# TheEconomist/us-potus-model

Hardware: AMD Instinct MI355X
Metric: leapfrog_steps_per_sec (higher is better)
Workload: dtype f64

## Files before the change

### us_potus_model_amd/csrc/potus_cluster.hpp

```cpp
#pragma once
#include "potus_nuts.hpp"
#include "potus_dpp.hpp"

#define CL_MAXDAYS 64
#define CL_MAXK 32
#define CL_DW4_MAXAVG 26
#define CL_AUX_SC1 16
#define CL_NCHUNK PT_NW
#define CL_SEG_SHIFT 64
#define CL_SPIN_LIMIT 8000000u
#ifndef CL_SPIN_SLEEP
#define CL_SPIN_SLEEP 1
#endif

enum { CP_D0 = 0, CP_ND, CP_P0, CP_NP, CP_E0, CP_NE, CP_R0, CP_NR, CP_NSUB, CP_NSEG, CP_WB,
       CP_O_WD, CP_O_MASK, CP_O_SUB, CP_O_SEGPTR, CP_O_SEGKIND, CP_O_SEGIDX, CP_O_WT, CP_E_SH, CP_NCELL, CP_O_CELL, CP_N = 24 };
#define CL_CELLS_PER_THREAD 2
#define CL_G_PAD 16
enum { XP_PRE = 0, XP_AR = 64, XP_S = 66, XP_P = 72 };
enum { XQ0 = 64 };

struct ClModel {
  int K, XW, NR, NREP, NDP, npmax, nsubmax, Dint;
  const int *part;
  const int *sched;
  const double *wt;
  const int *rep_pos;
  const int *rep_owner;
  const double *rep_scale;
  const int *perm;
  int GS, GROWS;
  int l_C, l_G, l_Lw, l_prior, l_pm, l_py, l_pun, l_sub, l_tab, l_ru, l_wide, l_wout, l_X, l_Y, l_r, l_rep, l_bT, l_e, l_c1, l_c2, l_c3, l_ge, l_P, l_scal, l_red, l_st, l_prof;
  int lds_doubles;
};
typedef const ClModel AS_C *CCp;

#define CL_WIDE 96
struct ClLay {
  int l_C, l_G, l_Lw, l_prior, l_pm, l_py, l_pun, l_sub, l_tab, l_ru, l_wide, l_wout, l_X, l_Y, l_r, l_rep, l_bT, l_e, l_c1, l_c2, l_c3, l_ge, l_P, l_scal, l_red, l_st, l_prof;
  int l_rm, l_rpf, l_rrs;
  int total;
};
constexpr int cl_ev(int n) { return (n + 1) & ~1; }
constexpr ClLay cl_layout(int S, int SE, int SP, int NDP, int npcap, int nsubcap, int nrepcap, int nrcap, int tcap, int g_doubles, int necap = 0) {
  ClLay L{};
  int o = 0;
  L.l_C = o; o += cl_ev(S * NDP);
  L.l_G = g_doubles ? o : 0; o += cl_ev(g_doubles);
  L.l_Lw = o; o += cl_ev((SE + 1) * SP);
  L.l_prior = o; o += cl_ev(SE);
  L.l_pm = o; o += cl_ev(npcap + 8);
  L.l_py = o; o += cl_ev(npcap + 8);
  L.l_pun = o; o += cl_ev(npcap + 8);
  L.l_sub = o; o += cl_ev(nsubcap * 4 + 4);
  L.l_tab = o; o += cl_ev((npcap + 64) / 2 + 2);
  L.l_ru = o; o += cl_ev(npcap + 2);
  L.l_wide = o; o += cl_ev(CL_WIDE * PT_NW);
  L.l_wout = o; o += cl_ev(CL_WIDE);
  L.l_X = o; o += cl_ev((PT_NW + 1) * SE);
  L.l_Y = o; o += cl_ev((PT_NW + 1) * SE > nsubcap ? (PT_NW + 1) * SE : nsubcap);
  L.l_r = o; o += cl_ev(npcap + 2);
  L.l_rep = o; o += cl_ev(nrepcap + 2);
  L.l_bT = o; o += cl_ev(SE);
  L.l_e = o; o += cl_ev(tcap);
  L.l_c1 = o; o += cl_ev(CL_MAXDAYS);
  L.l_c2 = o; o += cl_ev(CL_MAXDAYS);
  L.l_c3 = o; o += cl_ev(CL_MAXDAYS);
  L.l_ge = o; o += cl_ev(CL_MAXDAYS);
  L.l_P = o; o += cl_ev(nrcap + 8);
  L.l_scal = o; o += cl_ev(SC_N);
  L.l_red = o; o += cl_ev((PT_NW + 1) * PT_NRED);
  L.l_st = o; o += cl_ev((npcap + 8 + 7) / 8);
  L.l_prof = o; o += cl_ev(PT_NPROF);
  L.l_rm = necap ? o : 0; o += necap ? cl_ev(necap + 8) : 0;
  L.l_rpf = necap ? o : 0; o += necap ? cl_ev(necap + 8) : 0;
  L.l_rrs = necap ? o : 0; o += necap ? cl_ev(necap + 8) : 0;
  L.total = o;
  return L;
}

struct ClFixed {
  static constexpr int S = 51, SE = 52, SP = 51, NDP = 33;
  static constexpr int NPCAP = 256, NSUBCAP = 384, NREPCAP = 768, NRCAP = 512, TCAP = 320;
  static constexpr int KMAX = 16;
  static constexpr int NECAP = 1920;
  static constexpr int XW = 832;
  static constexpr int GS = 48, GROWS = 52;
  static constexpr ClLay L = cl_layout(S, SE, SP, NDP, NPCAP, NSUBCAP, NREPCAP, NRCAP, TCAP, 0, NECAP);
#define CLF(f) static constexpr int f = L.f
  CLF(l_C); CLF(l_G); CLF(l_Lw); CLF(l_prior); CLF(l_pm); CLF(l_py); CLF(l_pun); CLF(l_sub); CLF(l_tab); CLF(l_ru); CLF(l_wide); CLF(l_wout); CLF(l_X); CLF(l_Y);
  CLF(l_r); CLF(l_rep); CLF(l_bT); CLF(l_e); CLF(l_c1); CLF(l_c2); CLF(l_c3); CLF(l_ge); CLF(l_P); CLF(l_scal); CLF(l_red); CLF(l_st); CLF(l_prof); CLF(l_rm); CLF(l_rpf); CLF(l_rrs);
#undef CLF
  static constexpr int lds_doubles = L.total;
};
template <int TAG> struct ClTag {
  static constexpr int DW = (TAG == 12 || TAG == 16 || TAG == 17) ? 4 : TAG;
  static constexpr bool MF = TAG == 12;
  static constexpr bool FX = TAG == 16 || TAG == 17;
  static constexpr int FULL = TAG == 16 ? 1 : 0;
};
typedef const int AS_C *cip;

__device__ __forceinline__ double bld_s(rsrc_t r, unsigned voff, unsigned soff) {
  return __builtin_bit_cast(double, __builtin_amdgcn_raw_buffer_load_b64(r, voff, soff, CL_AUX_SC1));
}
__device__ __forceinline__ void bst_s(rsrc_t r, unsigned voff, unsigned soff, double v) {
  __builtin_amdgcn_raw_buffer_store_b64(__builtin_bit_cast(u32x2, v), r, voff, soff, CL_AUX_SC1);
}
__device__ __forceinline__ double readlane_d(double v, int l) {
  const unsigned long long u = __builtin_bit_cast(unsigned long long, v);
  const unsigned lo = __builtin_amdgcn_readlane((unsigned)u, l), hi = __builtin_amdgcn_readlane((unsigned)(u >> 32), l);
  return __builtin_bit_cast(double, ((unsigned long long)hi << 32) | lo);
}
template <class P> __device__ __forceinline__ P launder_s(P p) {
  unsigned lo = __builtin_amdgcn_readfirstlane((unsigned)(unsigned long long)p);
  unsigned hi = __builtin_amdgcn_readfirstlane((unsigned)((unsigned long long)p >> 32));
  asm volatile("" : "+s"(lo), "+s"(hi));
  return (P)(((unsigned long long)hi << 32) | lo);
}

#ifdef POTUS_PROF
#define PROFPTR prof
#define CPROFPTR(c) (c).prof
#else
#define PROFPTR nullptr
#define CPROFPTR(c) nullptr
#endif
#if defined(POTUS_PROF_FETCH) && (POTUS_PROF_FETCH + 0) == 2
#define XPROF_A(p) nullptr
#define XPROF_B(p) (p)
#elif defined(POTUS_PROF_FETCH)
#define XPROF_A(p) (p)
#define XPROF_B(p) nullptr
#else
#define XPROF_A(p) nullptr
#define XPROF_B(p) nullptr
#endif
__shared__ int cl_dead;
__shared__ int cl_local;
#define STORE128_PAD(w) asm volatile("s_nop 1" :: "v"(w) : "memory")
struct Xch {
  rsrc_t xb;
  unsigned epoch;
  unsigned launch;
  unsigned x1e;
  int K, m, XW;
  int local;
};
__device__ __forceinline__ unsigned xch_wslot(const Xch &x, int mm) { return ((((x.epoch + 1u) & 3u) * (unsigned)x.K + (unsigned)mm) * (unsigned)x.XW) * 16u; }
__device__ __forceinline__ unsigned xch_rslot(const Xch &x, int mm) { return (((x.epoch & 3u) * (unsigned)x.K + (unsigned)mm) * (unsigned)x.XW) * 16u; }
__device__ __forceinline__ unsigned xch_eslot(const Xch &x, unsigned e, int mm) { return (((e & 3u) * (unsigned)x.K + (unsigned)mm) * (unsigned)x.XW) * 16u; }
__device__ __forceinline__ unsigned xch_wdoff(const Xch &x) { return 4u * (unsigned)x.K * (unsigned)x.XW * 16u; }
__device__ __forceinline__ bool xch_watchdog_raised(const Xch &x) {
  return __builtin_amdgcn_readfirstlane(__builtin_amdgcn_raw_buffer_load_b32(x.xb, 0u, __builtin_amdgcn_readfirstlane(xch_wdoff(x)), CL_AUX_SC1)) != 0u;
}
__device__ __forceinline__ void xch_give_up(const Xch &x) {
  __builtin_amdgcn_raw_buffer_store_b32(1u, x.xb, 0u, __builtin_amdgcn_readfirstlane(xch_wdoff(x)), CL_AUX_SC1);
  cl_dead = 1;
  asm volatile("s_waitcnt vmcnt(0) lgkmcnt(0)" ::: "memory");
  __builtin_amdgcn_endpgm();
}
__device__ __forceinline__ void xst(const Xch &x, unsigned voff, double v) {
  const unsigned long long u = __builtin_bit_cast(unsigned long long, v);
  const u32x4 w = {(unsigned)u, (unsigned)(u >> 32), x.epoch + 1u, x.launch};
  const unsigned so = __builtin_amdgcn_readfirstlane(xch_wslot(x, x.m));
  __builtin_amdgcn_raw_buffer_store_b128(w, x.xb, x.local ? voff : PT_OOB, so, 0);
  __builtin_amdgcn_raw_buffer_store_b128(w, x.xb, x.local ? PT_OOB : voff, so, CL_AUX_SC1);
  STORE128_PAD(w);
}
template <int NB>
__device__ __forceinline__ bool xld(const Xch &x_in, const unsigned (&vo)[NB], const unsigned (&so)[NB], double (&out)[NB], unsigned tag = 0, ldp xprof = nullptr) {
  Xch x = x_in;
  if (tag) x.epoch = tag;
  x.epoch = __builtin_amdgcn_readfirstlane(x.epoch); x.launch = __builtin_amdgcn_readfirstlane(x.launch);
#ifdef POTUS_PROF_FETCH
  const long long xt0_ = clock64();
#else
  (void)xprof;
#endif
  u32x4 w[NB];
  bool done[NB];
  unsigned ss[NB];
#pragma unroll
  for (int u = 0; u < NB; u++) ss[u] = __builtin_amdgcn_readfirstlane(so[u]);
// ... 242 lines not shown
  static constexpr int NEXTRA = 3;
  double extra[3];
  struct QT { double q; };
  struct GT { double p, m, pp; };
  __device__ __forceinline__ void q_load(unsigned vo, QT &t) { t.q = bld(r, vo, sQc); }
  __device__ __forceinline__ void qs_load(unsigned vo, QT &t) { t.q = bld_s(r, vo, sQc); }
  __device__ __forceinline__ double q_fin(QT &t) { return t.q; }
  __device__ __forceinline__ void g_load(unsigned vo, GT &t) {
    t.p = bld(r, vo, sPH); t.m = bld(r, vo, sM);
    t.pp = bld(r, fuse1 ? vo : PT_OOB, sPrev);
  }
  template <bool SHARED>
  __device__ __forceinline__ double fin(unsigned vo, double v, double q, const GT &t) {
    const double pf = t.p + he * v;
    bst(r, vo, sL, pf);
    const double ph = pf + he * v;
    bst(r, vo, sPH, ph);
    const double qn = q + e * t.m * ph;
    if (SHARED) bst_s(r, vo, sQn, qn);
    else bst(r, vo, sQn, qn);
    const double rs = t.pp + pf;
    bst(r, fuse1 ? vo : PT_OOB, sOut1, rs);
    extra[0] += t.m * pf * pf;
    extra[1] += t.m * t.pp * rs;
    extra[2] += t.m * pf * rs;
    return qn;
  }
  __device__ __forceinline__ double g_fin(unsigned vo, double v, double q, const GT &t) { return fin<false>(vo, v, q, t); }
  __device__ __forceinline__ double gs_fin(unsigned vo, double v, double q, const GT &t) { return fin<true>(vo, v, q, t); }
};

struct ClLeapPolicyRes {
  rsrc_t r;
  unsigned sQc, sQn, sPH, sL;
  double he, e;
  unsigned sOut1;
  bool fuse1, out1_global;
  unsigned e0b;
  static constexpr int NEXTRA = 3;
  double extra[3];
  struct QT { double q; };
  struct GT { double p, m, pp; };
  __device__ __forceinline__ int slot(unsigned vo) const { return vo == PT_OOB ? (int)ClFixed::NECAP : (int)((vo - e0b) >> 3); }
  static __device__ __forceinline__ ldp RM() { return (ldp)lds_dyn + ClFixed::l_rm; }
  static __device__ __forceinline__ ldp RPF() { return (ldp)lds_dyn + ClFixed::l_rpf; }
  static __device__ __forceinline__ ldp RRS() { return (ldp)lds_dyn + ClFixed::l_rrs; }
  __device__ __forceinline__ void q_load(unsigned vo, QT &t) { t.q = bld(r, vo, sQc); }
  __device__ __forceinline__ void qs_load(unsigned vo, QT &t) { t.q = bld_s(r, vo, sQc); }
  __device__ __forceinline__ double q_fin(QT &t) { return t.q; }
  __device__ __forceinline__ void g_load(unsigned vo, GT &t) {
    t.p = bld(r, vo, sPH);
    const int idx = slot(vo);
    t.m = RM()[idx];
    const double ppv = RPF()[idx];
    t.pp = fuse1 ? ppv : 0.0;
  }
  template <bool SHARED>
  __device__ __forceinline__ double fin(unsigned vo, double v, double q, const GT &t) {
    const int idx = slot(vo);
    const bool ok = vo != PT_OOB;
    const double pf = t.p + he * v;
    bst(r, vo, sL, pf);
    RPF()[idx] = ok ? pf : 0.0;
    const double ph = pf + he * v;
    bst(r, vo, sPH, ph);
    const double qn = q + e * t.m * ph;
    if (SHARED) bst_s(r, vo, sQn, qn);
    else bst(r, vo, sQn, qn);
    const double rs = t.pp + pf;
    RRS()[idx] = ok ? rs : 0.0;
    bst(r, (fuse1 && out1_global) ? vo : PT_OOB, sOut1, rs);
    extra[0] += t.m * pf * pf;
    extra[1] += t.m * t.pp * rs;
    extra[2] += t.m * pf * rs;
    return qn;
  }
  __device__ __forceinline__ double g_fin(unsigned vo, double v, double q, const GT &t) { return fin<false>(vo, v, q, t); }
  __device__ __forceinline__ double gs_fin(unsigned vo, double v, double q, const GT &t) { return fin<true>(vo, v, q, t); }
};

struct ClStatic {
  int s2info;
  int wd0, wnd;
  int ca, cb;
  unsigned rep_vo[2];
  unsigned rep_xo[2];
  int sg_a, sg_b, sg_kind, sg_index;
  double scale_r;
  int cellw[CL_CELLS_PER_THREAD];
};

__device__ __forceinline__ ClStatic cl_load_static(CCp CL, cip part) {
  ClStatic c;
  gcip sc = as_g(CL->sched) + part[CP_O_WD];
  const int tid = threadIdx.x;
  c.s2info = sc[tid];
  c.wd0 = sc[PT_THREADS + (tid >> 6)]; c.wnd = sc[PT_THREADS + PT_NW + (tid >> 6)];
  c.ca = sc[PT_THREADS + 2 * PT_NW + (tid >> 6)]; c.cb = sc[PT_THREADS + 3 * PT_NW + (tid >> 6)];
  gcip rp = as_g(CL->rep_pos);
  const int NREP = CL->NREP;
  gcip ro = as_g(CL->rep_owner);
#pragma unroll
  for (int u = 0; u < 2; u++) {
    const int j = tid + u * PT_THREADS;
    c.rep_vo[u] = j < NREP ? 8u * (unsigned)rp[j] : PT_OOB;
    c.rep_xo[u] = j < NREP ? ((unsigned)ro[j] * (unsigned)CL->XW + (unsigned)(XQ0 + j)) * 16u : PT_OOB;
  }
  {
    gcip sch = as_g(CL->sched);
    const int nseg = part[CP_NSEG];
    const int sg = CL->l_G ? ((tid + PT_THREADS / 2) & (PT_THREADS - 1)) : ((tid + PT_THREADS - CL_SEG_SHIFT) & (PT_THREADS - 1));
    const bool ok = sg < nseg;
    c.sg_a = ok ? sch[part[CP_O_SEGPTR] + sg] : 0;
    c.sg_b = ok ? sch[part[CP_O_SEGPTR] + sg + 1] : 0;
    c.sg_kind = ok ? sch[part[CP_O_SEGKIND] + sg] : 3;
    c.sg_index = ok ? sch[part[CP_O_SEGIDX] + sg] : 0;
#pragma unroll
    for (int h = 0; h < CL_CELLS_PER_THREAD; h++) c.cellw[h] = CL->l_G ? sch[part[CP_O_CELL] + h * PT_THREADS + tid] : 0;
    const int jr = tid - 128;
    c.scale_r = (jr >= 0 && jr < part[CP_NR]) ? as_g(CL->rep_scale)[part[CP_R0] + jr] : 0.0;
  }
  return c;
}
__device__ __forceinline__ ClStatic cl_setup_lds(CMp M, CCp CL, cip part, ldp lds) {
  if (threadIdx.x == 0) { cl_dead = 0; cl_local = 0; }
#ifdef CL_POISON_LDS
  for (int i = threadIdx.x; i < CL->lds_doubles; i += PT_THREADS) lds[i] = __builtin_nan("");
  __syncthreads();
#endif
  ldp Lw = lds + CL->l_Lw;
  gcdp src = as_g(M->mat);
  for (int i = threadIdx.x; i < (M->SE + 1) * M->SP; i += PT_THREADS) Lw[i] = i < M->SE * M->SP ? src[i] : 0.0;
  for (int i = threadIdx.x; i < M->SE; i += PT_THREADS) (lds + CL->l_prior)[i] = src[M->m_priorx + i];
  unsigned char AS_L *st = (unsigned char AS_L *)(lds + CL->l_st);
  gcip ps = as_g(M->pi) + part[CP_P0];
  const int np = part[CP_NP];
  for (int i = threadIdx.x; i < np + 8; i += PT_THREADS) st[i] = i < np ? (unsigned char)ps[i] : (unsigned char)0;
  {
    unsigned long long AS_L *pm = (unsigned long long AS_L *)(lds + CL->l_pm);
    unsigned long long AS_L *pyn = (unsigned long long AS_L *)(lds + CL->l_py);
    ldp pun = lds + CL->l_pun;
    const int Npad = M->Npad, p0 = part[CP_P0], d0 = part[CP_D0], full = M->full;
    gcip pi = as_g(M->pi);
    gcdp pd = as_g(M->pd);
    for (int i = threadIdx.x; i < np + 8; i += PT_THREADS) {
      unsigned long long v = 0;
      double y = 0.0, N = 0.0, un = 0.0;
      if (i < np) {
        const int g = p0 + i;
        v = (unsigned long long)(unsigned)pi[g] | ((unsigned long long)(unsigned)(pi[Npad + g] - d0) << 8) |
            ((unsigned long long)(unsigned)pi[2 * Npad + g] << 16);
        if (full) v |= ((unsigned long long)(unsigned)pi[3 * Npad + g] << 32) | ((unsigned long long)(unsigned)pi[4 * Npad + g] << 40);
        {
          gcip scw = as_g(CL->sched) + part[CP_O_WD];
          const int tl_ = pi[Npad + g] - d0;
          int wt = 0;
          for (int w_ = 0; w_ < PT_NW; w_++) { const int a_ = scw[PT_THREADS + w_], n_ = scw[PT_THREADS + PT_NW + w_]; if (tl_ >= a_ && tl_ < a_ + n_) wt = w_; }
          v |= (unsigned long long)(unsigned)wt << 48;
        }
        y = pd[g]; N = pd[Npad + g]; un = full ? pd[2 * Npad + g] : 0.0;
      }
      pm[i] = v; pyn[i] = (unsigned long long)(unsigned)(int)y | ((unsigned long long)(unsigned)(int)N << 32); pun[i] = un;
    }
    unsigned AS_L *tab = (unsigned AS_L *)(lds + CL->l_tab);
    gcip src_tab = as_g(CL->sched) + part[CP_O_MASK];
    for (int i = threadIdx.x; i < np + 64; i += PT_THREADS) tab[i] = i < np ? (unsigned)src_tab[i] : 0u;
    unsigned short AS_L *sb = (unsigned short AS_L *)(lds + CL->l_sub);
    gcip src_sub = as_g(CL->sched) + part[CP_O_SUB];
    const int n16 = part[CP_NSUB] * PT_SUBLEN;
    for (int i = threadIdx.x; i < n16; i += PT_THREADS) sb[i] = (unsigned short)src_sub[i];
  }
  if (CL->l_G) for (int i = threadIdx.x; i < CL->GROWS * CL->GS + CL_G_PAD; i += PT_THREADS) (lds + CL->l_G)[i] = 0.0;
  const ClStatic c = cl_load_static(CL, part);
#ifdef POTUS_PROF
  for (int i = threadIdx.x; i < PT_NPROF; i += PT_THREADS) (lds + CL->l_prof)[i] = 0.0;
#endif
  __syncthreads();
  return c;
}

__device__ __forceinline__ int uni_i(int v) { return __builtin_amdgcn_readfirstlane(v); }

template <int CL_TAG, class Pol>
__device__ __forceinline__ double cl_pass_partial(CMp M_in, CCp CL_in, cip part_in, ldp lds, const ClStatic &cst, Xch &x, Pol &pol_io,
                                                  bool pubnext, const LeafCtx &pend, ltp ts, ldp wout, bool &aborted) {
  constexpr int CL_DW = ClTag<CL_TAG>::DW;
  constexpr bool MF = ClTag<CL_TAG>::MF, FX = ClTag<CL_TAG>::FX;
#define LAY(f) (FX ? (int)ClFixed::f : CL->f)
  Pol pol = pol_io;
  int tid = threadIdx.x;
  asm volatile("" : "+v"(tid));
  CMp M = launder_s(M_in);
  CCp CL = launder_s(CL_in);
  cip part = launder_s(part_in);
  const int lane = tid & 63;
  const int w = __builtin_amdgcn_readfirstlane(tid >> 6);
  if constexpr (FX) lds = (ldp)lds_dyn;
  const int S = FX ? (int)ClFixed::S : M->S, T = M->T, SE = FX ? (int)ClFixed::SE : M->SE, SP = FX ? (int)ClFixed::SP : M->SP, full = FX ? ClTag<CL_TAG>::FULL : M->full, o_c = M->o_c;
  const int NDP = FX ? (int)ClFixed::NDP : CL->NDP, NR = CL->NR, NREP = CL->NREP;
  const int d0 = part[CP_D0], nd = part[CP_ND], np = part[CP_NP], e0 = part[CP_E0], r0 = part[CP_R0], nr = part[CP_NR];
  const int K = x.K, m = x.m;
  const int wd0 = __builtin_amdgcn_readfirstlane(cst.wd0), wnd = __builtin_amdgcn_readfirstlane(cst.wnd);
  ldp C = lds + LAY(l_C), Lw = lds + LAY(l_Lw), X = lds + LAY(l_X), Y = lds + LAY(l_Y), r_lds = lds + LAY(l_r), ru_lds = lds + LAY(l_ru);
  ldp s_rep = lds + LAY(l_rep);
  ldp s_zT = s_rep, s_zb = s_rep + S, s_mid = s_rep + 2 * S;
  ldp s_bT = lds + LAY(l_bT), s_e = lds + LAY(l_e), s_c1 = lds + LAY(l_c1), s_c2 = lds + LAY(l_c2), s_c3 = lds + LAY(l_c3);
  ldp s_ge = lds + LAY(l_ge), s_P = lds + LAY(l_P), s_scal = lds + LAY(l_scal), red = lds + LAY(l_red);
  const int e_noise = e0 + S * nd, e_ze = part[CP_E_SH], e_rep = e_ze + (full ? nd : 0);
  double lp = 0.0;
#ifdef POTUS_PROF
  ldp prof = lds + LAY(l_prof);
#endif
  PROF_START();
  TSTAMP(0);

  double cs[CL_DW], zq[CL_DW];
  {
    typename Pol::QT qr[2], qt[CL_DW];
    const bool ahead = x.x1e != 0;
    pol.qs_load(ahead ? PT_OOB : cst.rep_vo[0], qr[0]);
    pol.qs_load(ahead ? PT_OOB : cst.rep_vo[1], qr[1]);
    double qx[2];
    {
      const unsigned vo[2] = {ahead ? cst.rep_xo[0] : PT_OOB, ahead ? cst.rep_xo[1] : PT_OOB};
      const unsigned so[2] = {xch_eslot(x, x.x1e, 0), xch_eslot(x, x.x1e, 0)};
      xld(x, vo, so, qx, ahead ? x.x1e : 1u);
    }
#pragma unroll
    for (int j = 0; j < CL_DW; j++) {
      const int tl = wd0 + j;
      pol.q_load((lane < S && j < wnd) ? 8u * (unsigned)(e0 + lane + S * tl) : PT_OOB, qt[j]);
    }
    for (int i = tid; i < NR + 8; i += PT_THREADS) s_P[i] = 0.0;
    if (tid >= 64 && tid < 64 + CL_MAXDAYS) s_ge[tid - 64] = 0.0;
#pragma unroll
    for (int u = 0; u < 2; u++) { const int j = tid + u * PT_THREADS; s_rep[j < NREP ? j : NREP] = ahead ? qx[u] : pol.q_fin(qr[u]); }
    double run = 0.0;
#pragma unroll
    for (int j = CL_DW - 1; j >= 0; j--) {
      const int t = d0 + wd0 + j;
      const double z = pol.q_fin(qt[j]);
      zq[j] = z;
      lp -= 0.5 * z * z;
      run += (t < T - 1) ? z : 0.0;
      cs[j] = run;
    }
    if (lane < S) {
      Y[w * SE + lane] = run;
#pragma unroll
      for (int j = 0; j < CL_DW; j++) { if (j < wnd) C[lane * NDP + wd0 + j] = cs[j]; }
    }
  }
  __syncthreads();
// ... 144 lines not shown
      s_scal[SC_DSRHO] = M->sigma_e * (-rho / sqrt(1.0 - rho * rho));
    }
    if (w == PT_NW - 2 && pend.n >= 0) {
      WPROF_T0B();
      WPROF_PTB(29);
      cl_leaf_logic(ts, pend, wout);
      WPROF_PTB(30);
    }
    const bool no_polls_here = w == PT_NW - 2 && pend.n >= 0 && np <= 64 * w;
    for (int i0 = 0; i0 < (no_polls_here ? 0 : np); i0 += PT_THREADS) {
      const int il = i0 + tid;
      const bool ok = il < np, lead = ok;
      const int ic = ok ? il : np;
      const unsigned vq = lead ? 8u * (unsigned)(e_noise + il) : PT_OOB;
      typename Pol::QT qt;
      typename Pol::GT gt;
      pol.q_load(vq, qt);
      pol.g_load(vq, gt);
      double gval = 0.0, zn = 0.0;
      if (i0 + 64 * w < np) {
        const unsigned long long meta = pm[ic];
        const int s = (int)(meta & 0xffu), tl = (int)((meta >> 8) & 0xffu), ip = (int)((meta >> 16) & 0xffffu);
        const int im = (int)((meta >> 32) & 0xffu), ipop = (int)((meta >> 40) & 0xffu);
        const unsigned long long yn = pyn[ic];
        const double y = (double)(int)(unsigned)yn, N = (double)(int)(unsigned)(yn >> 32), un = pun[ic];
        const int t = d0 + tl;
        ldp L0 = Lw + s * SP, C0 = C + tl, CW = X + (int)((meta >> 48) & 0xffu) * SE;
        double a0 = 0.0, a1 = 0.0;
          int k0 = 0;
          constexpr int DW_ = 10;
          for (; k0 + DW_ <= S; k0 += DW_) {
            double l[DW_], c[DW_], cw[DW_];
#pragma unroll
            for (int j = 0; j < DW_; j++) { l[j] = L0[k0 + j]; c[j] = C0[(k0 + j) * NDP]; cw[j] = CW[k0 + j]; }
            ISSUE_FENCE();
#pragma unroll
            for (int j = 0; j < DW_; j++) c[j] = c[j] + cw[j];
#pragma unroll
            for (int j = 0; j < DW_; j += 2) { a0 += l[j] * c[j]; a1 += l[j + 1] * c[j + 1]; }
          }
          for (; k0 < S; k0 += 4) {
            double l[4], c[4];
#pragma unroll
            for (int j = 0; j < 4; j++) { const int kk = min(k0 + j, S - 1); l[j] = L0[kk]; c[j] = C0[kk * NDP] + CW[kk]; }
            ISSUE_FENCE();
#pragma unroll
            for (int j = 0; j < 4; j += 2) {
              a0 += (k0 + j < S ? l[j] : 0.0) * c[j];
              a1 += (k0 + j + 1 < S ? l[j + 1] : 0.0) * c[j + 1];
            }
          }
        const double dot = a0 + a1;
        const double sg = s == S ? sigma_nn : sigma_ns;
        WPROF_CSTAMP(0);
        zn = pol.q_fin(qt);
#if (POTUS_PROF_CMASK & 2)
        __builtin_amdgcn_s_waitcnt(0x0F70);
#endif
        WPROF_CSTAMP(1);
        double eta = s_bT[s] + sg * zn + sigma_c * s_mid[ip] + dot;
        if (full) eta += sigma_m * s_mid[om + im] + sigma_pop * s_mid[opop + ipop] + un * s_e[t];
        const double ex = exp(-fabs(eta)), l1 = log1p(ex), pr = (eta >= 0.0 ? 1.0 : ex) / (1.0 + ex);
        const double r = y - N * pr;
        WPROF_CSTAMP(2);
        const double term = y * (fmin(eta, 0.0) - l1) + (N - y) * (fmin(-eta, 0.0) - l1) - 0.5 * zn * zn;
        lp += term;
        r_lds[lead ? il : np + 1] = r;
        ru_lds[lead ? il : np + 1] = r * un;
        gval = sg * r - zn;
      }
      pol.g_fin(vq, gval, zn, gt);
      WPROF_CSTAMP(3);
    }
    WPROF_CFLUSH();
  }
  WAVE_ARRIVE(3);
  __syncthreads();
  PROF_MARK(3);
  TSTAMP(4);
  if (pend.n >= 0 && uni_i(ts->abort)) { aborted = true; return 0.0; }

  if constexpr (!MF) {
    const unsigned AS_L *tab = (const unsigned AS_L *)(lds + LAY(l_tab));
    const int lk = lane < S ? lane : 0;
    const int ca = __builtin_amdgcn_readfirstlane(cst.ca), cb = __builtin_amdgcn_readfirstlane(cst.cb);
    double acc = 0.0;
    for (int base = ca; base < cb; base += 64) {
      const int mine = base + lane < cb ? base + lane : np;
      const unsigned ev = tab[mine];
      const double rv = r_lds[mine];
      const int cnt = min(64, cb - base);
      for (int p0 = 0; p0 < cnt; p0 += 8) {
        unsigned e8[8];
        double r8[8], l8[8];
#pragma unroll
        for (int u = 0; u < 8; u++) {
          const int pu = p0 + u;
          e8[u] = (unsigned)__builtin_amdgcn_readlane((int)ev, pu);
          r8[u] = readlane_d(rv, pu);
          l8[u] = Lw[(int)(e8[u] & 0xffu) * SP + lk];
        }
        ISSUE_FENCE();
#pragma unroll
        for (int u = 0; u < 8; u++) {
          acc += r8[u] * l8[u];
          if (e8[u] & 0x10000u) {
            if (lane < S) C[lane * NDP + (int)((e8[u] >> 8) & 0xffu)] = acc;
          }
        }
      }
    }
    if (lane < S) X[w * SE + lane] = acc;
  }
  if constexpr (MF) {
    ldp G = lds + LAY(l_G);
#pragma unroll
    for (int h = 0; h < CL_CELLS_PER_THREAD; h++) {
      if (h == 0 || part[CP_NCELL] > h * PT_THREADS) {
        const int cw = cst.cellw[h], a = cw & 1023, cnt = (cw >> 10) & 63, off = (int)((unsigned)cw >> 16);
        double sum = r_lds[a];
        for (int i = 1; i < cnt; i++) sum += r_lds[a + i];
        G[off] = sum;
      }
    }
  }
  {
    const int nsub = part[CP_NSUB], wb = part[CP_WB];
    const u32x4 AS_L *sb = (const u32x4 AS_L *)(lds + LAY(l_sub));
    for (int sub0 = 0; sub0 < nsub; sub0 += PT_THREADS) {
      const int sub = sub0 + tid;
      const bool ok = sub < nsub;
      const u32x4 ia = sb[ok ? 2 * sub : 0], ib = sb[ok ? 2 * sub + 1 : 0];
      double rr[PT_SUBLEN];
      ldp rsrc_ = sub >= wb ? ru_lds : r_lds;
#pragma unroll
      for (int j = 0; j < 4; j++) {
        rr[2 * j] = rsrc_[ok ? (int)(ia[j] & 0xffffu) : np]; rr[2 * j + 1] = rsrc_[ok ? (int)(ia[j] >> 16) : np];
        rr[8 + 2 * j] = rsrc_[ok ? (int)(ib[j] & 0xffffu) : np]; rr[9 + 2 * j] = rsrc_[ok ? (int)(ib[j] >> 16) : np];
      }
      ISSUE_FENCE();
      double sum = 0.0;
#pragma unroll
      for (int j = 0; j < PT_SUBLEN; j++) sum += rr[j];
      if (ok) Y[sub] = sum;
    }
  }
  WAVE_ARRIVE(4);
  __syncthreads();
  PROF_MARK(4);
  TSTAMP(5);

  int tlast[CL_DW], ch[CL_DW];
  double cv[CL_DW];
  double chunk_total = 0.0;
  if constexpr (!MF) {
#pragma unroll
    for (int j = 0; j < CL_DW; j++) {
      const int info = __builtin_amdgcn_readlane(cst.s2info, j);
      tlast[j] = (info & 0xff) - 1; ch[j] = info >> 8;
      cv[j] = C[(lane < S ? lane : 0) * NDP + max(tlast[j], 0)];
    }
    if (w == 0) {
      double ct[PT_NW];
      const int lx = lane < S ? lane : S;
#pragma unroll
      for (int c = 0; c < PT_NW; c++) ct[c] = X[c * SE + lx];
      ISSUE_FENCE();
#pragma unroll
      for (int c = 0; c < PT_NW; c++) ct[c] = lane < S ? ct[c] : 0.0;
#pragma unroll
      for (int c = 0; c < PT_NW; c++) { X[c * SE + lx] = chunk_total; chunk_total += ct[c]; }
    }
  } else {
    (void)tlast; (void)ch; (void)cv;
    if (w < 4) {
      ldp G = lds + LAY(l_G);
      const int GS = CL->GS, nst = CL->GROWS >> 2, g = lane >> 4, n = lane & 15;
      const int nt = (nd + 15) >> 4;
      double carry[4] = {0.0, 0.0, 0.0, 0.0};
      constexpr int NST = 16;
      for (int tt = 0; tt < nt; tt++) {
        typedef double d4_t __attribute__((ext_vector_type(4)));
        d4_t acc = {0.0, 0.0, 0.0, 0.0};
#pragma unroll
        for (int h0 = 0; h0 < NST; h0 += 8) {
          double av[8], bv[8];
#pragma unroll
          for (int u = 0; u < 8; u++) {
            const int st = h0 + u;
            av[u] = Lw[min(4 * st + g, SE) * SP + 16 * w + n];
            bv[u] = G[min(4 * st + g, 4 * nst - 1) * GS + 16 * tt + n];
          }
          ISSUE_FENCE();
#pragma unroll
          for (int u = 0; u < 8; u++) acc = __builtin_amdgcn_mfma_f64_16x16x4f64(av[u], bv[u], acc, 0, 0, 0);
          ISSUE_FENCE();
        }
#pragma unroll
        for (int v = 0; v < 4; v++) {
          double x = acc[v];
          x += dpp_fetch<DPP_ROW_SHR(1), 0xf>(0.0, x);
          x += dpp_fetch<DPP_ROW_SHR(2), 0xf>(0.0, x);
          x += dpp_fetch<DPP_ROW_SHR(4), 0xf>(0.0, x);
          x += dpp_fetch<DPP_ROW_SHR(8), 0xf>(0.0, x);
          x += carry[v];
          const int k = 16 * w + g + 4 * v, t = 16 * tt + n;
          if (k < S && t < nd) C[k * NDP + t] = x;
          const unsigned long long u = __builtin_bit_cast(unsigned long long, x);
          const unsigned lo = (unsigned)__builtin_amdgcn_ds_swizzle((int)(unsigned)u, 0x1f0), hi = (unsigned)__builtin_amdgcn_ds_swizzle((int)(unsigned)(u >> 32), 0x1f0);
          carry[v] = __builtin_bit_cast(double, ((unsigned long long)hi << 32) | lo);
        }
      }
    }
  }
  {
    double sum = 0.0;
    const int sg_a = cst.sg_a, sg_b = cst.sg_b, sg_kind = cst.sg_kind, sg_index = cst.sg_index;
    for (int j0 = sg_a; j0 < sg_b; j0 += 8) {
      double yy[8];
#pragma unroll
      for (int u = 0; u < 8; u++) yy[u] = Y[min(j0 + u, sg_b - 1)];
      ISSUE_FENCE();
#pragma unroll
      for (int u = 0; u < 8; u++) sum += j0 + u < sg_b ? yy[u] : 0.0;
    }
    if (sg_kind == 0) s_P[sg_index] = sum;
    else if (sg_kind == 2) s_ge[sg_index] = sum;
// ... 809 lines not shown
```

### us_potus_model_amd/csrc/potus_hmc.hip

```cpp
#include "../../include/potus_hmc.h"
#include "potus_nuts.hpp"
#include "potus_cluster.hpp"
#include "potus_nuts_twin.hpp"
#include "potus_dense.hpp"
#include "potus_summary.hpp"
#include "potus_diag.hpp"
#include "potus_monitor.hpp"

#include <algorithm>
#include <cmath>
#include <cstdarg>
#include <cstdio>
#include <cstdlib>
#include <cstring>
#include <limits>
#include <memory>
#include <charconv>
#include <chrono>
#include <thread>
#include <mutex>
#include <string>
#include <vector>


// ... 1375 lines not shown
        int tl = 0, worst = 0;
        for (int wv = 0; wv < PT_NW; wv++) {
          int n = 0, polls = 0;
          while (tl < nd && n < DW) {
            const int c1 = dp[d0 + tl + 1] - dp[d0 + tl];
            if (n > 0 && polls + c1 > B && (nd - tl) <= (PT_NW - 1 - wv) * DW) break;
            polls += c1; n++; tl++;
          }
          worst = std::max(worst, polls);
        }
        return tl == nd ? worst : 1 << 30;
      };
      int best = hi2, bestB = hi2;
      for (int B = lo2; B <= hi2; B++) { const int w_ = maxpolls(B); if (w_ < best) { best = w_; bestB = B; } }
      if (!assign(bestB, true)) return fail(POTUS_ERR_STATE, "internal: member %d: %d days do not fit %d waves", m, nd, PT_NW);
    }
    std::vector<int> ca(PT_NW), cb(PT_NW), tab(np), s2info(PT_THREADS, 0);
    for (int wv = 0; wv < PT_NW; wv++) { ca[wv] = (int)((long long)np * std::min(wv, CL_NCHUNK) / CL_NCHUNK); cb[wv] = (int)((long long)np * std::min(wv + 1, CL_NCHUNK) / CL_NCHUNK); }
    auto chunk_of = [&](int il) { int c = 0; while (c < CL_NCHUNK - 1 && il >= cb[c]) c++; return c; };
    for (int il = 0; il < np; il++) {
      const int g = p0 + il, tl = sp->h_pt[g] - d0;
      const bool dayend = il == np - 1 || sp->h_pt[g + 1] != sp->h_pt[g];
      tab[il] = sp->h_ps[g] | (tl << 8) | ((dayend ? 1 : 0) << 16);
    }
    for (int wv = 0; wv < PT_NW; wv++)
      for (int j = 0; j < wnd[wv]; j++) {
        int tl = wd0[wv] + j;
        while (tl >= 0 && dp[d0 + tl + 1] == dp[d0 + tl]) tl--;
        s2info[wv * 64 + j] = tl < 0 ? 0 : ((tl + 1) | (chunk_of(dp[d0 + tl + 1] - 1 - p0) << 8));
      }
    std::vector<int> cellw((size_t)CL_CELLS_PER_THREAD * PT_THREADS, 0);
    int ncell = 0;
    if (mfma) {
      const int dump = GROWS * GS;
      if (np >= 1024) return fail(POTUS_ERR_UNSUPPORTED, "cluster mode: member %d has %d polls (the adjoint scatter addresses 1023)", m, np);
      for (auto &cw : cellw) cw = np | (1 << 10) | (dump << 16);
      for (int il = 0; il < np;) {
        int j = il + 1;
        while (j < np && sp->h_pt[p0 + j] == sp->h_pt[p0 + il] && sp->h_ps[p0 + j] == sp->h_ps[p0 + il]) j++;
        {
          if (j - il > 63) return fail(POTUS_ERR_UNSUPPORTED, "cluster mode: %d polls of one state on one day (the adjoint scatter takes 63)", j - il);
          if (ncell >= CL_CELLS_PER_THREAD * PT_THREADS) return fail(POTUS_ERR_UNSUPPORTED, "cluster mode: member %d has more than %d polled (state, day) cells", m, CL_CELLS_PER_THREAD * PT_THREADS);
          cellw[ncell++] = il | ((j - il) << 10) | ((sp->h_ps[p0 + il] * GS + (sp->h_pt[p0 + il] - d0)) << 16);
        }
        il = j;
      }
    }
    pt_[CP_NCELL] = ncell;
    std::vector<int> wdays(wd0);
    wdays.insert(wdays.end(), wnd.begin(), wnd.end());
    wdays.insert(wdays.end(), ca.begin(), ca.end());
    wdays.insert(wdays.end(), cb.begin(), cb.end());

    std::vector<int> sub16, seg_ptr{0}, seg_kind, seg_index;
    std::vector<double> sub_wt;
    int nsub = 0;
    auto add_group = [&](int nseg, int kind, int index0, bool weighted, auto key) {
      std::vector<std::vector<int>> lists(nseg);
      for (int il = 0; il < np; il++) lists[key(p0 + il)].push_back(il);
      for (int sgi = 0; sgi < nseg; sgi++) {
        const auto &l = lists[sgi];
        if (l.empty()) continue;
        for (size_t a = 0; a < l.size(); a += PT_SUBLEN) {
          for (size_t j = a; j < a + PT_SUBLEN; j++) {
            sub16.push_back(j < l.size() ? l[j] : np);
            if (weighted) sub_wt.push_back(j < l.size() ? sp->h_pu[p0 + l[j]] : 0.0);
          }
          nsub++;
        }
        seg_ptr.push_back(nsub);
        seg_kind.push_back(kind); seg_index.push_back(index0 + sgi);
      }
    };
    add_group(P, 0, 2 * S, false, [&](int i) { return sp->h_pp[i]; });
    if (full) {
      add_group(M.M, 0, 2 * S + P, false, [&](int i) { return sp->h_pm[i]; });
      add_group(M.Pop, 0, 2 * S + P + M.M, false, [&](int i) { return sp->h_ppop[i]; });
    }
    const int wb = nsub;
    if (full) add_group(nd, 2, 0, false, [&](int i) { return sp->h_pt[i] - d0; });
    seg_ptr.push_back(nsub);
    if ((int)seg_kind.size() > PT_THREADS) return fail(POTUS_ERR_UNSUPPORTED, "cluster mode: member %d has %zu segments (> %d)", m, seg_kind.size(), PT_THREADS);
    pt_[CP_NSUB] = nsub; pt_[CP_NSEG] = (int)seg_kind.size(); pt_[CP_WB] = wb;
    nsubmax = std::max(nsubmax, nsub);
    auto appi = [&](const std::vector<int> &v) {
      while (sched.size() % 4) sched.push_back(0);
      const int off = (int)sched.size();
      sched.insert(sched.end(), v.begin(), v.end());
      return off;
    };
    pt_[CP_O_WD] = appi(s2info); appi(wdays);
    pt_[CP_O_MASK] = appi(tab); pt_[CP_O_SUB] = appi(sub16); pt_[CP_O_SEGPTR] = appi(seg_ptr);
    pt_[CP_O_SEGKIND] = appi(seg_kind); pt_[CP_O_SEGIDX] = appi(seg_index);
    pt_[CP_O_CELL] = appi(cellw);
    while (wts.size() % 2) wts.push_back(0.0);
    pt_[CP_O_WT] = (int)wts.size();
    wts.insert(wts.end(), sub_wt.begin(), sub_wt.end());
  }
  const int Dint = e;
  C.Dint = Dint;
  for (int k = 0; k < 16; k++) { sched.push_back(0); wts.push_back(0.0); }
  C.npmax = npmax; C.nsubmax = nsubmax;

  std::vector<int> iperm(L.D, -1);
  for (int i = 0; i < Dint; i++) { if (perm[i] >= L.D) return fail(POTUS_ERR_STATE, "internal: bad permutation"); if (perm[i] >= 0) iperm[perm[i]] = i; }
  for (int i = 0; i < L.D; i++) if (iperm[i] < 0) return fail(POTUS_ERR_STATE, "internal: cluster layout misses parameter %d", i);
  std::vector<int> rep_pos(C.NREP), rep_owner(C.NREP);
  for (int j = 0; j < C.NREP; j++) {
    rep_pos[j] = iperm[j < S ? L.o_zT + j : j < 2 * S ? L.o_zb + (j - S) : L.o_c + (j - 2 * S)];
    int mo = 0;
    while (mo < K - 1 && rep_pos[j] >= part[(size_t)mo * CP_N + CP_E0] + part[(size_t)mo * CP_N + CP_NE]) mo++;
    rep_owner[j] = mo;
  }
  std::vector<double> rep_scale(C.NR, 1.0);
  for (int i = 0; i < S; i++) { rep_scale[i] = M.aT; rep_scale[S + i] = M.aB; }
  for (int i = 0; i < P; i++) rep_scale[2 * S + i] = d->sigma_c;
  if (full) {
    for (int i = 0; i < M.M; i++) rep_scale[2 * S + P + i] = d->sigma_m;
    for (int i = 0; i < M.Pop; i++) rep_scale[2 * S + P + M.M + i] = d->sigma_pop;
  }
  sp->h_perm = perm;

  int ndmax = 1, nemax = 0;
  for (int m = 0; m < K; m++) { ndmax = std::max(ndmax, part[(size_t)m * CP_N + CP_ND]); nemax = std::max(nemax, part[(size_t)m * CP_N + CP_NE]); }
  C.NDP = ndmax | 1;
  C.GS = GS; C.GROWS = GROWS;
  ClLay lay = cl_layout(S, M.SE, M.SP, C.NDP, npmax, nsubmax, C.NREP, C.NR, T, mfma ? GROWS * GS + CL_G_PAD : 0);
  {
    const bool fits = DW == 4 && !mfma && K <= ClFixed::KMAX && std::max(XP_P + C.NR, XQ0 + C.NREP) <= ClFixed::XW && S == ClFixed::S && M.SE == ClFixed::SE && M.SP == ClFixed::SP && ndmax <= ClFixed::NDP - 1 && npmax <= ClFixed::NPCAP &&
                      nsubmax <= ClFixed::NSUBCAP && C.NREP <= ClFixed::NREPCAP && C.NR <= ClFixed::NRCAP && T <= ClFixed::TCAP && (int)SC_N <= 8 &&
                      nemax <= ClFixed::NECAP;
    if (fits && !(getenv("POTUS_CL_DYNAMIC") && atoi(getenv("POTUS_CL_DYNAMIC")))) {
      C.NDP = ClFixed::NDP; C.XW = ClFixed::XW;
      lay = ClFixed::L;
      sp->cl_dw = full ? 16 : 17;
    }
  }
  C.l_C = lay.l_C; C.l_G = lay.l_G; C.l_Lw = lay.l_Lw; C.l_prior = lay.l_prior; C.l_pm = lay.l_pm; C.l_py = lay.l_py; C.l_pun = lay.l_pun;
  C.l_sub = lay.l_sub; C.l_tab = lay.l_tab; C.l_ru = lay.l_ru; C.l_wide = lay.l_wide; C.l_wout = lay.l_wout; C.l_X = lay.l_X; C.l_Y = lay.l_Y;
  C.l_r = lay.l_r; C.l_rep = lay.l_rep; C.l_bT = lay.l_bT; C.l_e = lay.l_e; C.l_c1 = lay.l_c1; C.l_c2 = lay.l_c2; C.l_c3 = lay.l_c3; C.l_ge = lay.l_ge;
  C.l_P = lay.l_P; C.l_scal = lay.l_scal; C.l_red = lay.l_red; C.l_st = lay.l_st; C.l_prof = lay.l_prof; C.lds_doubles = lay.total;
  const int o = lay.total;
  sp->cl_lds_bytes = (size_t)o * 8 + sizeof(TS) + 16;
  if (sp->cl_lds_bytes > 160 * 1024 - 64) return fail(POTUS_ERR_UNSUPPORTED, "cluster mode needs %zu bytes of LDS per workgroup", sp->cl_lds_bytes);

  int rc;
  if ((rc = upload(sp, part, &C.part)) || (rc = upload(sp, sched, &C.sched)) || (rc = upload(sp, wts, &C.wt)) ||
      (rc = upload(sp, rep_pos, &C.rep_pos)) || (rc = upload(sp, rep_owner, &C.rep_owner)) || (rc = upload(sp, rep_scale, &C.rep_scale)) || (rc = upload(sp, perm, &C.perm)))
    return rc;
  void *pc = nullptr;
  HIP_TRY(hipMalloc(&pc, sizeof(ClModel)));
  sp->allocs.push_back(pc);
  HIP_TRY(hipMemcpy(pc, &C, sizeof(ClModel), hipMemcpyHostToDevice));
  sp->dCL = (ClModel *)pc;
  for (const void *f : {reinterpret_cast<const void *>(k_cl_logprob_grad<4>), reinterpret_cast<const void *>(k_cl_logprob_grad<8>), reinterpret_cast<const void *>(k_cl_logprob_grad<12>),
                        reinterpret_cast<const void *>(k_cl_logprob_grad<16>), reinterpret_cast<const void *>(k_cl_init<16>),
                        reinterpret_cast<const void *>(k_cl_run<16, false>), reinterpret_cast<const void *>(k_cl_run<16, true>),
                        reinterpret_cast<const void *>(k_cl_logprob_grad<17>), reinterpret_cast<const void *>(k_cl_init<17>),
                        reinterpret_cast<const void *>(k_cl_run<17, false>), reinterpret_cast<const void *>(k_cl_run<17, true>),
                        reinterpret_cast<const void *>(k_cl_init<4>), reinterpret_cast<const void *>(k_cl_init<8>), reinterpret_cast<const void *>(k_cl_init<12>),
                        reinterpret_cast<const void *>(k_cl_run<4, false>), reinterpret_cast<const void *>(k_cl_run<8, false>), reinterpret_cast<const void *>(k_cl_run<12, false>),
                        reinterpret_cast<const void *>(k_cl_run<4, true>), reinterpret_cast<const void *>(k_cl_run<8, true>), reinterpret_cast<const void *>(k_cl_run<12, true>)})
    HIP_TRY(hipFuncSetAttribute(f, hipFuncAttributeMaxDynamicSharedMemorySize, (int)sp->cl_lds_bytes));
  sp->K = K;
  return 0;
}

#define CL_DISPATCH(tag, CALL) do { if ((tag) == 16) { CALL(16); } else if ((tag) == 17) { CALL(17); } else if ((tag) == 4) { CALL(4); } else if ((tag) == 12) { CALL(12); } else { CALL(8); } } while (0)

int read_scalars(Sampler *sp, std::vector<ChainScalars> &sc) {
  std::vector<ChainScalars> all((size_t)sp->R.chains * sp->K);
  HIP_TRY(hipMemcpy(all.data(), sp->R.scal, sizeof(ChainScalars) * all.size(), hipMemcpyDeviceToHost));
  sc.resize(sp->R.chains);
  for (int c = 0; c < sp->R.chains; c++) sc[c] = all[(size_t)c * sp->K];
  return 0;
}

int check_chains(Sampler *sp) {
  std::vector<ChainScalars> sc;
  { const int rc_ = read_scalars(sp, sc); if (rc_) return rc_; }
  if (sp->coop()) {
    const size_t per_chain = 4 * (size_t)sp->K * sp->CL.XW + 8;
    for (int b = 0; b < sp->R.chains * sp->sides(); b++) {
      const int c = b % sp->R.chains;
      unsigned wd = 0, wt = 0;
      HIP_TRY(hipMemcpy(&wd, (const char *)sp->R.xbuf + ((size_t)b * per_chain + 4 * (size_t)sp->K * sp->CL.XW) * 16, 4, hipMemcpyDeviceToHost));
      if (sp->twin) HIP_TRY(hipMemcpy(&wt, (const char *)sp->R.twbuf + ((size_t)c * TWB_WORDS + TWB_WD) * 16, 4, hipMemcpyDeviceToHost));
      wd |= wt;
      if (wd) return fail(POTUS_ERR_WATCHDOG, "chain %d: the %d workgroups working for it were not running together (is another process using GPU %d?); "
                                              "the launch was abandoned and this handle is no longer usable", c + 1, sp->K * sp->sides(), sp->device);
    }
  }
  for (int c = 0; c < sp->R.chains; c++) {
    if (sp->n_ds && (sc[c].status == POTUS_ERR_INIT || sc[c].status == POTUS_ERR_STEPSIZE)) continue;
    if (sc[c].status == POTUS_ERR_INIT) return fail(POTUS_ERR_INIT, "chain %d: no finite initial log density/gradient after 100 attempts", c + 1);
    if (sc[c].status == POTUS_ERR_STEPSIZE) return fail(POTUS_ERR_STEPSIZE, "chain %d: the step-size search left (0, 1e7) -- the posterior is improper or the gradient is wrong (Stan throws here)", c + 1);
    if (sc[c].status == POTUS_ERR_WATCHDOG) return fail(POTUS_ERR_WATCHDOG, "chain %d: cluster launch abandoned (watchdog)", c + 1);
    if (sc[c].status != 0) return fail(POTUS_ERR_STATE, "chain %d: status %d", c + 1, sc[c].status);
  }
  return 0;
}


int dense_window_capacity(int nw, int ib, int tb, int bw) {
  if (nw < 20) return 1;
  int cap = 1, n = 0, counter = 0, next = ib + bw - 1, size = bw;
  for (int it = 0; it < nw; it++) {
    const bool in = counter >= ib && counter < nw - tb && counter != nw, end = counter == next && counter != nw;
// ... 3390 lines not shown
```

Before: 653,700.

## Precompute byte offsets in gather table and specialize fixed-build walk loops

The tab entries are rewritten at setup into packed byte offsets for the Lw row and the C column. Polls that should not store are redirected to an extra dump column in C, so the inner loop loses its branch and index arithmetic. The fixed builds use one unrolled pass over at most 32 polls (a group of 16, then conditional groups of 8). The level-1 task array is padded with dummy indices so the per-lane bounds checks disappear. Per-wave ca/cb and nsub/wb now come from s2info lanes via readlane instead of extra scalar fields, which adds LDS padding, a 16-bit offset limit, and new host-side packing.

```diff
diff --git a/us_potus_model_amd/csrc/potus_cluster.hpp b/us_potus_model_amd/csrc/potus_cluster.hpp
--- a/us_potus_model_amd/csrc/potus_cluster.hpp
+++ b/us_potus_model_amd/csrc/potus_cluster.hpp
@@ -7,6 +7,10 @@
 #define CL_DW4_MAXAVG 26
 #define CL_AUX_SC1 16
 #define CL_NCHUNK PT_NW
+#define CL_WALK_FX0 16
+#define CL_WALK_FX1 8
+#define CL_WALK_GROUP 16
+#define CL_L1_LANE 32
 #define CL_SEG_SHIFT 64
 #define CL_SPIN_LIMIT 8000000u
 #ifndef CL_SPIN_SLEEP
@@ -42,17 +46,19 @@
   int total;
 };
 constexpr int cl_ev(int n) { return (n + 1) & ~1; }
+constexpr int cl_subpad(int nsub) { return nsub > PT_THREADS ? (nsub + PT_THREADS - 1) / PT_THREADS * PT_THREADS : PT_THREADS; }
+constexpr int cl_ndp(int ndmax) { return (ndmax + 1) | 1; }
 constexpr ClLay cl_layout(int S, int SE, int SP, int NDP, int npcap, int nsubcap, int nrepcap, int nrcap, int tcap, int g_doubles, int necap = 0) {
   ClLay L{};
   int o = 0;
-  L.l_C = o; o += cl_ev(S * NDP);
+  L.l_C = o; o += cl_ev(S * NDP + NDP + 64);
   L.l_G = g_doubles ? o : 0; o += cl_ev(g_doubles);
   L.l_Lw = o; o += cl_ev((SE + 1) * SP);
   L.l_prior = o; o += cl_ev(SE);
   L.l_pm = o; o += cl_ev(npcap + 8);
   L.l_py = o; o += cl_ev(npcap + 8);
   L.l_pun = o; o += cl_ev(npcap + 8);
-  L.l_sub = o; o += cl_ev(nsubcap * 4 + 4);
+  L.l_sub = o; o += cl_ev(cl_subpad(nsubcap) * 4 + 4);
   L.l_tab = o; o += cl_ev((npcap + 64) / 2 + 2);
   L.l_ru = o; o += cl_ev(npcap + 2);
   L.l_wide = o; o += cl_ev(CL_WIDE * PT_NW);
@@ -92,6 +98,7 @@
   CLF(l_r); CLF(l_rep); CLF(l_bT); CLF(l_e); CLF(l_c1); CLF(l_c2); CLF(l_c3); CLF(l_ge); CLF(l_P); CLF(l_scal); CLF(l_red); CLF(l_st); CLF(l_prof); CLF(l_rm); CLF(l_rpf); CLF(l_rrs);
 #undef CLF
   static constexpr int lds_doubles = L.total;
+  static_assert(NDP == cl_ndp(32) && NPCAP <= 32 * CL_NCHUNK && NSUBCAP <= PT_THREADS, "phase D of the fixed builds: 32 days and a dump column, chunks of at most 32 polls, one trip of level-1 tasks");
 };
 template <int TAG> struct ClTag {
   static constexpr int DW = (TAG == 12 || TAG == 16 || TAG == 17) ? 4 : TAG;
@@ -100,6 +107,7 @@
   static constexpr int FULL = TAG == 16 ? 1 : 0;
 };
 typedef const int AS_C *cip;
+template <int N> struct ClInt { static constexpr int value = N; };
 
 __device__ __forceinline__ double bld_s(rsrc_t r, unsigned voff, unsigned soff) {
   return __builtin_bit_cast(double, __builtin_amdgcn_raw_buffer_load_b64(r, voff, soff, CL_AUX_SC1));
@@ -508,7 +516,6 @@
 struct ClStatic {
   int s2info;
   int wd0, wnd;
-  int ca, cb;
   unsigned rep_vo[2];
   unsigned rep_xo[2];
   int sg_a, sg_b, sg_kind, sg_index;
@@ -522,7 +529,6 @@
   const int tid = threadIdx.x;
   c.s2info = sc[tid];
   c.wd0 = sc[PT_THREADS + (tid >> 6)]; c.wnd = sc[PT_THREADS + PT_NW + (tid >> 6)];
-  c.ca = sc[PT_THREADS + 2 * PT_NW + (tid >> 6)]; c.cb = sc[PT_THREADS + 3 * PT_NW + (tid >> 6)];
   gcip rp = as_g(CL->rep_pos);
   const int NREP = CL->NREP;
   gcip ro = as_g(CL->rep_owner);
@@ -537,10 +543,12 @@
     const int nseg = part[CP_NSEG];
     const int sg = CL->l_G ? ((tid + PT_THREADS / 2) & (PT_THREADS - 1)) : ((tid + PT_THREADS - CL_SEG_SHIFT) & (PT_THREADS - 1));
     const bool ok = sg < nseg;
-    c.sg_a = ok ? sch[part[CP_O_SEGPTR] + sg] : 0;
-    c.sg_b = ok ? sch[part[CP_O_SEGPTR] + sg + 1] : 0;
-    c.sg_kind = ok ? sch[part[CP_O_SEGKIND] + sg] : 3;
-    c.sg_index = ok ? sch[part[CP_O_SEGIDX] + sg] : 0;
+    const int sgl = ok ? sg : 0;
+    const int sa_ = sch[part[CP_O_SEGPTR] + sgl], sb_ = sch[part[CP_O_SEGPTR] + sgl + 1], sk_ = sch[part[CP_O_SEGKIND] + sgl], si_ = sch[part[CP_O_SEGIDX] + sgl];
+    c.sg_a = ok ? sa_ : 0;
+    c.sg_b = ok ? sb_ : 0;
+    c.sg_kind = ok ? sk_ : 3;
+    c.sg_index = ok ? si_ : 0;
 #pragma unroll
     for (int h = 0; h < CL_CELLS_PER_THREAD; h++) c.cellw[h] = CL->l_G ? sch[part[CP_O_CELL] + h * PT_THREADS + tid] : 0;
     const int jr = tid - 128;
@@ -590,11 +598,15 @@
     }
     unsigned AS_L *tab = (unsigned AS_L *)(lds + CL->l_tab);
     gcip src_tab = as_g(CL->sched) + part[CP_O_MASK];
-    for (int i = threadIdx.x; i < np + 64; i += PT_THREADS) tab[i] = i < np ? (unsigned)src_tab[i] : 0u;
+    const unsigned tab_dump = (unsigned)(CL->NDP - 1) * 8u << 16;
+    for (int i = threadIdx.x; i < np + 64; i += PT_THREADS) {
+      const unsigned hw = i < np ? (unsigned)src_tab[i] : 0u;
+      tab[i] = (hw & 0xffu) * (unsigned)M->SP * 8u | ((hw & 0x10000u) ? ((hw >> 8) & 0xffu) * 8u << 16 : tab_dump);
+    }
     unsigned short AS_L *sb = (unsigned short AS_L *)(lds + CL->l_sub);
     gcip src_sub = as_g(CL->sched) + part[CP_O_SUB];
-    const int n16 = part[CP_NSUB] * PT_SUBLEN;
-    for (int i = threadIdx.x; i < n16; i += PT_THREADS) sb[i] = (unsigned short)src_sub[i];
+    const int n16 = part[CP_NSUB] * PT_SUBLEN, n16pad = cl_subpad(part[CP_NSUB]) * PT_SUBLEN;
+    for (int i = threadIdx.x; i < n16pad; i += PT_THREADS) sb[i] = (unsigned short)(i < n16 ? src_sub[i] : np);
   }
   if (CL->l_G) for (int i = threadIdx.x; i < CL->GROWS * CL->GS + CL_G_PAD; i += PT_THREADS) (lds + CL->l_G)[i] = 0.0;
   const ClStatic c = cl_load_static(CL, part);
@@ -905,32 +917,44 @@
 
   if constexpr (!MF) {
     const unsigned AS_L *tab = (const unsigned AS_L *)(lds + LAY(l_tab));
-    const int lk = lane < S ? lane : 0;
-    const int ca = __builtin_amdgcn_readfirstlane(cst.ca), cb = __builtin_amdgcn_readfirstlane(cst.cb);
+    const int ca = __builtin_amdgcn_readlane(cst.s2info, CL_L1_LANE + 1), cb = __builtin_amdgcn_readlane(cst.s2info, CL_L1_LANE + 2);
+    const char AS_L *Lw_me = (const char AS_L *)(Lw + (lane < S ? lane : 0));
+    char AS_L *C_me = (char AS_L *)(C + (lane < S ? lane * NDP : S * NDP + (lane - S)));
     double acc = 0.0;
-    for (int base = ca; base < cb; base += 64) {
-      const int mine = base + lane < cb ? base + lane : np;
+    auto walk = [&](unsigned ev, double rv, int p0, auto gw) {
+      constexpr int G = decltype(gw)::value;
+      unsigned e[G];
+      double r[G], l[G];
+#pragma unroll
+      for (int u = 0; u < G; u++) {
+        const int pu = p0 + u;
+        e[u] = (unsigned)__builtin_amdgcn_readlane((int)ev, pu);
+        r[u] = readlane_d(rv, pu);
+        l[u] = *(const double AS_L *)(Lw_me + (e[u] & 0xffffu));
+      }
+      ISSUE_FENCE();
+#pragma unroll
+      for (int u = 0; u < G; u++) {
+        acc += r[u] * l[u];
+        *(double AS_L *)(C_me + (e[u] >> 16)) = acc;
+      }
+    };
+    if constexpr (FX) {
+      const int cnt = cb - ca;
+      const int mine = lane < cnt ? ca + lane : np;
       const unsigned ev = tab[mine];
       const double rv = r_lds[mine];
-      const int cnt = min(64, cb - base);
-      for (int p0 = 0; p0 < cnt; p0 += 8) {
-        unsigned e8[8];
-        double r8[8], l8[8];
-#pragma unroll
-        for (int u = 0; u < 8; u++) {
-          const int pu = p0 + u;
-          e8[u] = (unsigned)__builtin_amdgcn_readlane((int)ev, pu);
-          r8[u] = readlane_d(rv, pu);
-          l8[u] = Lw[(int)(e8[u] & 0xffu) * SP + lk];
-        }
-        ISSUE_FENCE();
-#pragma unroll
-        for (int u = 0; u < 8; u++) {
-          acc += r8[u] * l8[u];
-          if (e8[u] & 0x10000u) {
-            if (lane < S) C[lane * NDP + (int)((e8[u] >> 8) & 0xffu)] = acc;
-          }
-        }
+      walk(ev, rv, 0, ClInt<CL_WALK_FX0>());
+#pragma unroll
+      for (int p0 = CL_WALK_FX0; p0 < 32; p0 += CL_WALK_FX1)
+        if (cnt > p0) walk(ev, rv, p0, ClInt<CL_WALK_FX1>());
+    } else {
+      for (int base = ca; base < cb; base += 64) {
+        const int mine = base + lane < cb ? base + lane : np;
+        const unsigned ev = tab[mine];
+        const double rv = r_lds[mine];
+        const int cnt = min(64, cb - base);
+        for (int p0 = 0; p0 < cnt; p0 += CL_WALK_GROUP) walk(ev, rv, p0, ClInt<CL_WALK_GROUP>());
       }
     }
     if (lane < S) X[w * SE + lane] = acc;
@@ -948,24 +972,23 @@
     }
   }
   {
-    const int nsub = part[CP_NSUB], wb = part[CP_WB];
+    const int l1 = __builtin_amdgcn_readlane(cst.s2info, CL_L1_LANE), nsub = l1 & 0xffff, wb = (int)((unsigned)l1 >> 16);
     const u32x4 AS_L *sb = (const u32x4 AS_L *)(lds + LAY(l_sub));
-    for (int sub0 = 0; sub0 < nsub; sub0 += PT_THREADS) {
+    for (int sub0 = 0; sub0 < (FX ? 1 : nsub); sub0 += PT_THREADS) {
       const int sub = sub0 + tid;
-      const bool ok = sub < nsub;
-      const u32x4 ia = sb[ok ? 2 * sub : 0], ib = sb[ok ? 2 * sub + 1 : 0];
+      const u32x4 ia = sb[2 * sub], ib = sb[2 * sub + 1];
       double rr[PT_SUBLEN];
       ldp rsrc_ = sub >= wb ? ru_lds : r_lds;
 #pragma unroll
       for (int j = 0; j < 4; j++) {
-        rr[2 * j] = rsrc_[ok ? (int)(ia[j] & 0xffffu) : np]; rr[2 * j + 1] = rsrc_[ok ? (int)(ia[j] >> 16) : np];
-        rr[8 + 2 * j] = rsrc_[ok ? (int)(ib[j] & 0xffffu) : np]; rr[9 + 2 * j] = rsrc_[ok ? (int)(ib[j] >> 16) : np];
+        rr[2 * j] = rsrc_[(int)(ia[j] & 0xffffu)]; rr[2 * j + 1] = rsrc_[(int)(ia[j] >> 16)];
+        rr[8 + 2 * j] = rsrc_[(int)(ib[j] & 0xffffu)]; rr[9 + 2 * j] = rsrc_[(int)(ib[j] >> 16)];
       }
       ISSUE_FENCE();
       double sum = 0.0;
 #pragma unroll
       for (int j = 0; j < PT_SUBLEN; j++) sum += rr[j];
-      if (ok) Y[sub] = sum;
+      if (sub < nsub) Y[sub] = sum;
     }
   }
   WAVE_ARRIVE(4);
diff --git a/us_potus_model_amd/csrc/potus_hmc.hip b/us_potus_model_amd/csrc/potus_hmc.hip
--- a/us_potus_model_amd/csrc/potus_hmc.hip
+++ b/us_potus_model_amd/csrc/potus_hmc.hip
@@ -1481,6 +1481,12 @@
     seg_ptr.push_back(nsub);
     if ((int)seg_kind.size() > PT_THREADS) return fail(POTUS_ERR_UNSUPPORTED, "cluster mode: member %d has %zu segments (> %d)", m, seg_kind.size(), PT_THREADS);
     pt_[CP_NSUB] = nsub; pt_[CP_NSEG] = (int)seg_kind.size(); pt_[CP_WB] = wb;
+    static_assert(CL_L1_LANE >= 8 && CL_L1_LANE + 2 < 64, "lanes 0-7 of s2info are the wave's days");
+    if (nsub > 0xffff) return fail(POTUS_ERR_UNSUPPORTED, "cluster mode: member %d has %d level-1 tasks (> 65535)", m, nsub);
+    for (int wv = 0; wv < PT_NW; wv++) {
+      int *sl = &s2info[wv * 64 + CL_L1_LANE];
+      sl[0] = nsub | (wb << 16); sl[1] = ca[wv]; sl[2] = cb[wv];
+    }
     nsubmax = std::max(nsubmax, nsub);
     auto appi = [&](const std::vector<int> &v) {
       while (sched.size() % 4) sched.push_back(0);
@@ -1522,7 +1528,8 @@
 
   int ndmax = 1, nemax = 0;
   for (int m = 0; m < K; m++) { ndmax = std::max(ndmax, part[(size_t)m * CP_N + CP_ND]); nemax = std::max(nemax, part[(size_t)m * CP_N + CP_NE]); }
-  C.NDP = ndmax | 1;
+  C.NDP = cl_ndp(ndmax);
+  if (M.SE * M.SP * 8 > 0x10000 || C.NDP * 8 > 0x10000) return fail(POTUS_ERR_UNSUPPORTED, "cluster mode: the gather program holds byte offsets in 16 bits");
   C.GS = GS; C.GROWS = GROWS;
   ClLay lay = cl_layout(S, M.SE, M.SP, C.NDP, npmax, nsubmax, C.NREP, C.NR, T, mfma ? GROWS * GS + CL_G_PAD : 0);
   {
```

After: 660,500 (median of 6 runs). 1.1% higher.
